# cnuns/Com-MARL

Hardware: AMD Instinct MI355X
Metric: env-steps/sec (whole node), PredatorPrey M=10 N=4, 4096 envs at 1/2/4/8 GPUs (higher is better)
Workload: dtype f32

## Files before the change

com-marl_amd/csrc/cm_env_pp10_dev.h:

```cpp
#pragma once
#include "cm_env_dev.h"

namespace cm {
namespace pp10 {

constexpr int S = 10, N = 4, M = 4, D = 21;
constexpr uint32_t ONES = 0x01010101u, HIGH = 0x80808080u, LOW7 = 0x7f7f7f7fu, SIXTEENS = 0x10101010u;

__device__ __forceinline__ uint32_t cell_of(int r, int c) { return (uint32_t)((r + 1) * 16 + c + 1); }
__device__ __forceinline__ int row_of(uint32_t ci) { return (int)(ci >> 4) - 1; }
__device__ __forceinline__ int col_of(uint32_t ci) { return (int)(ci & 15u) - 1; }
__device__ __forceinline__ uint32_t byte_at(uint32_t w, int i) { return (w >> (8 * i)) & 0xffu; }
__device__ __forceinline__ uint32_t set_byte(uint32_t w, int i, uint32_t v) { return (w & ~(0xffu << (8 * i))) | (v << (8 * i)); }
__device__ __forceinline__ uint32_t bcast(uint32_t t) { return t * ONES; }
__device__ __forceinline__ uint32_t any0(uint32_t x) { return (x - ONES) & ~x & HIGH; }
__device__ __forceinline__ uint32_t zero_bytes(uint32_t x) { return ~(((x & LOW7) + LOW7) | x | LOW7); }
__device__ __forceinline__ uint32_t delta_of(int a) { return (uint32_t)(16 * dr_of(a) + dc_of(a)); }
__device__ __forceinline__ int inside(uint32_t t) { return (((t >> 4) - 1u) < 10u) & (((t & 15u) - 1u) < 10u); }
__device__ __forceinline__ int lacks(uint32_t layer, uint32_t t) { return any0(layer ^ bcast(t)) == 0u; }
__device__ __forceinline__ uint32_t live_preys(uint32_t ppos, uint32_t flags) {
    uint32_t w = ppos;
#pragma unroll
    for (int j = 0; j < M; ++j) w |= ((flags >> j) & 1u) ? 0u : (0xffu << (8 * j));
    return w;
}
__device__ __forceinline__ int count_next(uint32_t layer, uint32_t t) {
    return __popc(zero_bytes(layer ^ bcast(t - 16u)) | zero_bytes(layer ^ bcast(t - 1u)) | zero_bytes(layer ^ bcast(t + 1u)) |
                  zero_bytes(layer ^ bcast(t + 16u)));
}
struct Shifted { uint32_t m16, m1, p1, p16; };
__device__ __forceinline__ int agents_next(const Shifted &a, uint32_t t) {
    const uint32_t bt = bcast(t);
    return __popc(zero_bytes(a.m16 ^ bt) | zero_bytes(a.m1 ^ bt) | zero_bytes(a.p1 ^ bt) | zero_bytes(a.p16 ^ bt));
}
__device__ __forceinline__ int no_agent_next(const Shifted &a, uint32_t t) {
    const uint32_t bt = bcast(t);
    return (any0(a.m16 ^ bt) | any0(a.m1 ^ bt) | any0(a.p1 ^ bt) | any0(a.p16 ^ bt)) == 0u;
}

struct State { uint32_t apos, ppos, flags; };
struct Pre { uint32_t rng_step; int step_count_in, succ; float t_rc, t_step0, t_step; double t_rew; };

__device__ __forceinline__ uint32_t elem_code(int k) {
    const int i = k / D, f = k - D * i;
    int x;
    if (f < 18) { const int chn = f >= 9, w = f - 9 * chn, wr = w / 3, wc = w - 3 * wr; x = (wr * 16 + wc) | (chn << 6); }
    else x = 35 + (f - 18);
    return (uint32_t)(i | (x << 2));
}
struct Emit { uint32_t e0, e1; };
__device__ __forceinline__ Emit emit_codes(int sl) {
    Emit e{ 0u, 0u };
#pragma unroll
    for (int u = 0; u < 6; ++u) {
        const int k = min(16 * u + sl, N * D - 1);
        const uint32_t c = elem_code(k) << (10 * (u % 3));
        if (u < 3) e.e0 |= c; else e.e1 |= c;
    }
    return e;
}

__device__ __forceinline__ State load_state(const EnvDev &p, int b) {
    State s{ 0u, 0u, 0u };
#pragma unroll
    for (int i = 0; i < N; ++i) {
        const int2 q = p.agent_pos[(size_t)b * N + i];
        s.apos |= cell_of(q.x, q.y) << (8 * i);
        s.flags |= (p.agent_cond[(size_t)b * N + i] != 0 ? 16u : 0u) << i;
    }
#pragma unroll
    for (int j = 0; j < M; ++j) {
        const int2 q = p.prey_pos[(size_t)b * M + j];
        s.ppos |= cell_of(q.x, q.y) << (8 * j);
        s.flags |= (p.alive[(size_t)b * M + j] != 0 ? 1u : 0u) << j;
    }
    return s;
}
__device__ __forceinline__ Pre load_pre(const EnvDev &p, int b, int sl, int tx) {
    Pre e;
    e.step_count_in = p.step_count[b];
    e.succ = p.success[b];
    e.rng_step = p.rng_step[b];
    const int s0 = sl < S ? sl : S - 1;
    e.t_rc = (tx & 16) ? p.lut_col[s0] : p.lut_row[s0];
    e.t_step0 = p.lut_step[0];
    e.t_rew = p.rew_lut[sl < (M + 1) + (N + 1) ? sl : 0];
    const int sc = e.step_count_in + 1;
    e.t_step = p.lut_step[sc <= p.max_steps ? sc : p.max_steps];
    return e;
}

struct StepOff { uint32_t obs, reward, reward_f64, done, details, prey_alive, success, path_len; };
template <class T>
__device__ __forceinline__ T *at32(T *base, uint32_t elem) { return reinterpret_cast<T *>(reinterpret_cast<char *>(base) + (uint32_t)(elem * (uint32_t)sizeof(T))); }

__device__ __forceinline__ void write_back(const EnvDev &p, uint32_t b, int sl, uint32_t apos, uint32_t ppos, uint32_t flags, int step_count,
                                           int succ, uint32_t rng_step) {
    if (sl == 0) {
        *at32(p.rng_step, b) = rng_step;
        *at32(p.step_count, b) = step_count;
        *at32(p.success, b) = succ;
    }
    if (sl < M) {
        const uint32_t ca = byte_at(apos, sl), cp = byte_at(ppos, sl);
        *at32(p.agent_pos, b * N + sl) = make_int2(row_of(ca), col_of(ca));
        *at32(p.prey_pos, b * M + sl) = make_int2(row_of(cp), col_of(cp));
        *at32(p.alive, b * M + sl) = (uint8_t)((flags >> sl) & 1u);
    }
}

__device__ __forceinline__ void step(const EnvDev &p, State &st, Pre &pre, const Emit em, int act_off, const cm_step_out &out,
                                     const StepOff &off, bool last, int grp, int b_raw, bool grp_live, int lds_base, bool all_valid,
                                     int obs_copy) {
    Grp<16> g;
    const int tx = thread_x();
    g.sub = (tx & (WAVE - 1)) / 16; g.sl = tx % 16;
    const int sl = g.sl;
    ENV_PROBE(0);
    const bool valid = all_valid || (grp_live && b_raw < p.B);
    const int b = valid ? b_raw : p.B - 1;
    const Rng rng{ (uint32_t)(p.env_id_offset + b), pre.rng_step, p.key0, p.key1 };
    const bool mine = sl < M;
    u32x4 x0 = { 0, 0, 0, 0 };
    if (mine) x0 = rng.at(SITE_PREY, (uint32_t)(2 * sl));
    const int4 araw = *reinterpret_cast<const int4 *>(smem + act_off);
    const int ain[4] = { araw.x, araw.y, araw.z, araw.w };
    int act[4], bad = 0;
#pragma unroll
    for (int i = 0; i < N; ++i) {
        const int a = ain[i];
        const int bi = (unsigned)a > 4u;
        bad |= bi;
        const int faulty = ((st.flags >> (4 + i)) & 1u) == 0u;
        act[i] = bi ? 4 : ((faulty & (a != 4)) ? 5 : a);
    }
    if (bad && valid) {
        if (sl == 0) raise(p, CM_ERR_ACTION);
        write_back(p, (uint32_t)b, sl, st.apos, st.ppos, st.flags, pre.step_count_in, pre.succ, pre.rng_step);
    }
    const bool commit = valid && !bad;
    ENV_PROBE(1);
    ENV_PROBE(2);

    uint32_t apos = st.apos, ppos = st.ppos, flags = st.flags;
    uint32_t plive = live_preys(ppos, flags);
    int moving = 0;
#pragma unroll
    for (int i = 0; i < N; ++i) {
        const int a = act[i];
        const int active = a != 4;
        moving += active;
        const uint32_t t = byte_at(apos, i) + delta_of(a);
        const int ok = active & inside(t) & lacks(apos, t) & lacks(plive, t);
        apos = ok ? set_byte(apos, i, t) : apos;
    }
    ENV_PROBE(3);
    const Shifted ag{ apos - SIXTEENS, apos - ONES, apos + ONES, apos + SIXTEENS };
    int pk;
    {
        const uint32_t my = byte_at(ppos, sl & 3);
        const int my_alive = mine & (int)((flags >> (sl & 3)) & 1u);
        const int cnt = my_alive ? agents_next(ag, my) : 0;
        int mv = 4;
        int found = (my_alive ^ 1) | ((p.load == 2) & (cnt >= 2));
#pragma unroll
        for (int t = 0; t < 4; ++t) {
            const int m = prey_move_from_u32(pick(x0, t));
            const int ok = no_agent_next(ag, my + delta_of(m)) & (found ^ 1);
            mv = ok ? m : mv; found |= ok;
        }
        if (!found) {
            const u32x4 x1 = rng.at(SITE_PREY, (uint32_t)(2 * sl + 1));
            const int m = prey_move_from_u32(x1.x);
            mv = no_agent_next(ag, my + delta_of(m)) ? m : mv;
        }
        pk = cnt | (mv << 3);
    }
    ENV_PROBE(8);
    const int wsum = g.count(mine && count_next(plive, byte_at(apos, sl & 3)) != 0);
    int pks[M];
#pragma unroll
    for (int j = 0; j < M; ++j) pks[j] = __shfl(pk, j, 16);
    ENV_PROBE(4);
    int capture = 0, penalty = 0, alive_any = 0;
#pragma unroll
    for (int j = 0; j < M; ++j) {
        const uint32_t c = byte_at(ppos, j);
        const int alive = (int)((flags >> j) & 1u), cnt = pks[j] & 7, mv = pks[j] >> 3;
        int need = p.load;
        if (p.load != 2) {
            const uint32_t rf = c >> 4, cf = c & 15u;
            const int on_r = (rf == 1u) | (rf == (uint32_t)S), on_c = (cf == 1u) | (cf == (uint32_t)S);
            const int adj = (on_r & on_c) ? 2 : ((on_r | on_c) ? 3 : p.load);
            const int avail = adj - count_next(plive, c);
            need = p.load < avail ? p.load : avail;
        }
        const int hit = alive & (cnt >= 1), captured = hit & (need <= cnt);
        capture += captured; penalty += hit & (captured ^ 1);
        const int stays = alive & (captured ^ 1);
        const uint32_t t = c + delta_of(mv);
        const int ok = stays & (mv != 4) & inside(t) & lacks(apos, t) & lacks(plive, t);
        ppos = ok ? set_byte(ppos, j, t) : ppos;
        plive = stays ? (ok ? set_byte(plive, j, t) : plive) : (plive | (0xffu << (8 * j)));
        flags = stays ? flags : (flags & ~(1u << j));
        alive_any |= stays;
    }
    ENV_PROBE(5);
    double reward = __shfl(pre.t_rew, capture, 16) + __shfl(pre.t_rew, (M + 1) + moving, 16);
    if (p.load == 2) reward = reward + p.penalty * (double)penalty;
    const cm_step_out &o = out;
    const uint32_t ub = (uint32_t)b;
    if (commit && mine) *at32(o.prey_alive, off.prey_alive + ub * M + sl) = (uint8_t)((flags >> sl) & 1u);
    int step_count = pre.step_count_in + 1, succ = pre.succ;
    int done = (step_count >= p.max_steps) || !alive_any;
    if (done) succ = alive_any ? 0 : 1;
    if (step_count >= p.mpl) done = 1;
    if (sl == 0 && commit) {
        *at32(o.reward, off.reward + ub) = (float)reward;
        *at32(o.reward_f64, off.reward_f64 + ub) = reward;
        *at32(o.done, off.done + ub) = (uint8_t)done;
        *at32(o.path_len, off.path_len + ub) = done ? step_count : 0;
        int2 *dd = reinterpret_cast<int2 *>(at32(o.details, off.details + ub * 6));
        dd[0] = make_int2(capture, moving); dd[1] = make_int2(penalty, 0); dd[2] = make_int2(wsum, 0);
    }
    ENV_PROBE(6);
    if (__any(done)) {
        const Lds l = make_lds(S, N, M, lds_base + p.lds_env * grp, p.status);
        do_reset<CM_PP, 16>(p, l, rng, cm_rng_tape{}, b, g, done != 0);
        if (done) {
            uint32_t a = 0u, q = 0u;
#pragma unroll
            for (int i = 0; i < N; ++i) { a |= cell_of(AR(l, i), AC(l, i)) << (8 * i); q |= cell_of(PR(l, i), PC(l, i)) << (8 * i); }
            apos = a; ppos = q;
            flags |= 0x0fu;
        }
    }
    if (done) step_count = 0;
    ENV_PROBE(7);
    const float t_clock = done ? pre.t_step0 : pre.t_step;
    plive = live_preys(ppos, flags);
    float vv[6];
    int ci_copy[6];
#pragma unroll
    for (int u = 0; u < 6; ++u) {
        const uint32_t code = ((u < 3 ? em.e0 : em.e1) >> (10 * (u % 3))) & 0x1ffu;
        const uint32_t i = code & 3u, x = code >> 2, w = x & 63u;
        const uint32_t ci = (apos >> (8u * i)) & 0xffu;
        const uint32_t t = ci + w - 17u;
        const int hit = !lacks((x & 64u) ? plive : apos, t);
        const float tab = __shfl(pre.t_rc, x == 36u ? 16 + col_of(ci) : row_of(ci), 64);
        vv[u] = w < 35u ? (hit ? 1.0f : 0.0f) : (x == 37u ? t_clock : tab);
        ci_copy[u] = 16 * u + sl + 3 * (int)i;
    }
    st.apos = apos; st.ppos = ppos; st.flags = (commit && done) ? (flags | 0xf0u) : flags;
    pre.rng_step += 1u;
    if (commit) { pre.step_count_in = step_count; pre.succ = succ; }
    {
        const int sc = pre.step_count_in + 1;
        pre.t_step = p.lut_step[sc <= p.max_steps ? sc : p.max_steps];
    }
    if (!commit) return;
    if (sl == 0) *at32(o.success, off.success + ub) = succ;
    const uint32_t ob = off.obs + ub * (N * D) + (uint32_t)sl;
    float *oc = reinterpret_cast<float *>(smem + obs_copy);
#pragma unroll
    for (int u = 0; u < 6; ++u) {
        if (16 * u + sl < N * D) {
            *at32(o.obs, ob + 16u * u) = vv[u];
            oc[ci_copy[u]] = vv[u];
        }
    }
    static_assert(OBS_COPY_STRIDE == D + 3, "the copy index k + 3i assumes rows of 24 floats");
    if (last) write_back(p, ub, sl, apos, ppos, flags, step_count, succ, rng.step + 1);
    ENV_PROBE(9);
}

}
}
```

com-marl_amd/csrc/cm_policy_w_dev.h:

```cpp
#pragma once
#include <type_traits>

#include "cm_policy_h_dev.h"

namespace cm {
namespace mw {

using mf::FwdArgs;
using mf::v4f;
using mf::fast_tanh;
using mf::EH; using mf::EMB; using mf::H1; using mf::H2; using mf::H3; using mf::MAX_ACT;
using mh::v8h; using mh::v4h; using mh::h16;

constexpr int WG_ENVS = 16, WG_ROWS = 64, KH = 32;
constexpr int FRAG = 64;

struct PackW { int enc1, enc2, attn, gcn, x1, h3, h4, bias, lds_u4, h2, total; };
__host__ __device__ constexpr int frag_u4(int K, int OUT) { return (OUT / 16) * (K / 32) * 2 * FRAG; }
constexpr int BIAS_U4 = 144;
__host__ __device__ constexpr PackW pack_w(int L) {
    PackW o{};
    int off = 0;
    o.enc1 = off; off += frag_u4(KH, EH);
    o.enc2 = off; off += frag_u4(EH, EMB);
    o.attn = off; off += frag_u4(EMB, EMB);
    o.gcn = off; off += L * frag_u4(EMB, EMB);
    o.x1 = off; off += frag_u4(EMB, H1);
    o.h3 = off; off += frag_u4(H2, H3);
    o.h4 = off; off += frag_u4(H3, 32);
    o.bias = off; off += BIAS_U4;
    o.lds_u4 = off;
    o.h2 = off; off += frag_u4(H1, H2);
    o.total = off;
    return o;
}

struct BiasMap { int e1, e2, g, b1, b2, b3, b4, total; };
__host__ __device__ constexpr BiasMap bias_map(int L) {
    BiasMap o{};
    int off = 0;
    o.e1 = off; off += EH; o.e2 = off; off += EMB; o.g = off; off += (L > 0 ? L : 1) * EMB;
    o.b1 = off; off += H1; o.b2 = off; off += H2; o.b3 = off; off += H3; o.b4 = off; off += 32;
    o.total = off;
    return o;
}
__host__ __device__ inline size_t lds_policy_bytes(int L) { return (size_t)pack_w(L).lds_u4 * 16 + WG_ROWS * 4; }

struct WeightsW {
    const uint4 *pack;
    int n_act;
};

__host__ __device__ inline int kmap(int q, int g, int e) { return 32 * q + 16 * (e >> 2) + 4 * g + (e & 3); }

template <int KB> struct Act { v8h hi[KB], lo[KB]; };

#define CM_MFW(A, B, ACC) ACC = __builtin_amdgcn_mfma_f32_16x16x32_f16(A, B, ACC, 0, 0, 0)

template <int KB, int CT>
struct Frags {
    v8h h[CT][KB], l[CT][KB];
    template <int TAG = 0>
    __device__ __forceinline__ void fetch(const uint4 *W, int lane) {
#pragma unroll
        for (int ct = 0; ct < CT; ++ct)
#pragma unroll
            for (int q = 0; q < KB; ++q) {
                h[ct][q] = __builtin_bit_cast(v8h, W[((ct * KB + q) * 2 + 0) * FRAG + lane]);
                l[ct][q] = __builtin_bit_cast(v8h, W[((ct * KB + q) * 2 + 1) * FRAG + lane]);
            }
        __builtin_amdgcn_sched_barrier(0);
    }
};

template <int CT, bool ON>
struct BiasR {
    v4f b[ON ? CT : 1];
    template <int C0 = 0>
    __device__ __forceinline__ void fetch(const float *bias, int g) {
        if constexpr (ON) {
#pragma unroll
            for (int ct = C0; ct < CT; ++ct) { const float4 v = *reinterpret_cast<const float4 *>(bias + 16 * ct + 4 * g); b[ct] = (v4f){ v.x, v.y, v.z, v.w }; }
            __builtin_amdgcn_sched_barrier(0);
        }
    }
    __device__ __forceinline__ const v4f *regs() const { return ON ? b : nullptr; }
};
struct NoHook { __device__ __forceinline__ void operator()() const {} };

constexpr float TANH_PRESCALE = 2.8853900817779268f;

template <int N>
__device__ __forceinline__ void tanh_stage(float (&v)[N]) {
    float e[N];
#pragma unroll
    for (int i = 0; i < N; ++i) e[i] = __builtin_amdgcn_exp2f(v[i]);
#pragma unroll
    for (int i = 0; i < N; ++i) e[i] += 1.0f;
#pragma unroll
    for (int i = 0; i < N; ++i) e[i] = __builtin_amdgcn_rcpf(e[i]);
#pragma unroll
    for (int i = 0; i < N; ++i) v[i] = fmaf(-2.0f, e[i], 1.0f);
}
typedef _Float16 v2h __attribute__((ext_vector_type(2)));
typedef float v2f __attribute__((ext_vector_type(2)));
__host__ __device__ inline void split_u(float x, h16 &h, h16 &l) { h = (h16)x; l = (h16)(x - (float)h); }
enum { SPLIT_SUB = 0, SPLIT_MIX = 1, SPLIT_MIXLO = 2 };
constexpr int SPLIT_DEFAULT = SPLIT_MIXLO;
__device__ __forceinline__ float opaque_minus_one() { float m; asm("s_mov_b32 %0, -1.0" : "=s"(m)); return m; }
template <int N, int MODE = SPLIT_DEFAULT>
__device__ __forceinline__ void split_stage(const float (&y)[N], h16 (&h)[N], h16 (&l)[N]) {
    static_assert(N % 2 == 0, "pairs");
    float d[N];
#pragma unroll
    for (int i = 0; i < N; i += 2) { const v2h p = __builtin_convertvector((v2f){ y[i], y[i + 1] }, v2h); h[i] = p[0]; h[i + 1] = p[1]; }
    if constexpr (MODE == SPLIT_MIXLO) {
        const float m1 = opaque_minus_one();
#pragma unroll
        for (int i = 0; i < N; ++i) l[i] = (h16)__builtin_fmaf((float)h[i], m1, y[i]);
        return;
    }
    if constexpr (MODE == SPLIT_MIX) {
        const float m1 = opaque_minus_one();
#pragma unroll
        for (int i = 0; i < N; ++i) d[i] = __builtin_fmaf((float)h[i], m1, y[i]);
    } else {
#pragma unroll
        for (int i = 0; i < N; ++i) d[i] = y[i] - (float)h[i];
    }
#pragma unroll
    for (int i = 0; i < N; i += 2) { const v2h p = __builtin_convertvector((v2f){ d[i], d[i + 1] }, v2h); l[i] = p[0]; l[i + 1] = p[1]; }
}

template <int KB, int CT, bool TANH, bool BIAS, int SPLIT = SPLIT_DEFAULT, int PB0 = CT, class MID = NoHook>
__device__ __forceinline__ void dense_act(const Frags<KB, CT> &f, const float *bias, const Act<KB> &x, Act<CT / 2> &y, v4f *keep, int lane,
                                          float *sv = nullptr, const v4f *pb = nullptr, MID mid = MID{}) {
    const int g = lane >> 4;
    const v4f zero = (v4f){ 0.f, 0.f, 0.f, 0.f };
    v4f acc[CT];
#pragma unroll
    for (int p = 0; p <= CT / 2; ++p) {
        if constexpr (!std::is_same<MID, NoHook>::value) { if (p == CT / 4) mid(); }
        if (p < CT / 2) {
#pragma unroll
            for (int t = 0; t < 2; ++t) {
                const int ct = 2 * p + t;
                if (BIAS && ct >= PB0) acc[ct] = pb[ct];
                else if (BIAS) { const float4 b = *reinterpret_cast<const float4 *>(bias + 16 * ct + 4 * g); acc[ct] = (v4f){ b.x, b.y, b.z, b.w }; }
#pragma unroll
                for (int q = 0; q < KB; ++q) {
                    const v4f a0 = (q == 0 && !BIAS) ? zero : acc[ct];
                    acc[ct] = __builtin_amdgcn_mfma_f32_16x16x32_f16(f.h[ct][q], x.lo[q], a0, 0, 0, 0);
                    acc[ct] = __builtin_amdgcn_mfma_f32_16x16x32_f16(f.l[ct][q], x.hi[q], acc[ct], 0, 0, 0);
                    acc[ct] = __builtin_amdgcn_mfma_f32_16x16x32_f16(f.h[ct][q], x.hi[q], acc[ct], 0, 0, 0);
                }
            }
        }
        if (p > 0) {
            float v[8];
#pragma unroll
            for (int e = 0; e < 8; ++e) v[e] = acc[2 * (p - 1) + (e >> 2)][e & 3];
            if (TANH) tanh_stage<8>(v);
            if (keep) {
#pragma unroll
                for (int e = 0; e < 8; ++e) keep[2 * (p - 1) + (e >> 2)][e & 3] = v[e];
            }
            if (sv) {
                *reinterpret_cast<float4 *>(sv + 16 * (2 * (p - 1)) + 4 * g) = make_float4(v[0], v[1], v[2], v[3]);
                *reinterpret_cast<float4 *>(sv + 16 * (2 * (p - 1) + 1) + 4 * g) = make_float4(v[4], v[5], v[6], v[7]);
            }
            h16 h[8], l[8];
            split_stage<8, SPLIT>(v, h, l);
#pragma unroll
            for (int e = 0; e < 8; ++e) { y.hi[p - 1][e] = h[e]; y.lo[p - 1][e] = l[e]; }
        }
    }
}

template <int KB, int CT, bool SWAP, bool BIAS, bool PREB = false>
__device__ __forceinline__ void dense_f32(const Frags<KB, CT> &f, const float *bias, const Act<KB> &x, v4f (&out)[CT], int lane, const v4f *pb = nullptr) {
    const int g = lane >> 4;
    const v4f zero = (v4f){ 0.f, 0.f, 0.f, 0.f };
#pragma unroll
    for (int ct = 0; ct < CT; ++ct) {
        v4f acc = zero;
        if constexpr (BIAS && PREB) acc = pb[ct];
        else if (BIAS) { const float4 b = *reinterpret_cast<const float4 *>(bias + 16 * ct + 4 * g); acc = (v4f){ b.x, b.y, b.z, b.w }; }
#pragma unroll
        for (int q = 0; q < KB; ++q) {
            if (!SWAP) {
                acc = __builtin_amdgcn_mfma_f32_16x16x32_f16(f.h[ct][q], x.lo[q], acc, 0, 0, 0);
                acc = __builtin_amdgcn_mfma_f32_16x16x32_f16(f.l[ct][q], x.hi[q], acc, 0, 0, 0);
                acc = __builtin_amdgcn_mfma_f32_16x16x32_f16(f.h[ct][q], x.hi[q], acc, 0, 0, 0);
            } else {
                acc = __builtin_amdgcn_mfma_f32_16x16x32_f16(x.lo[q], f.h[ct][q], acc, 0, 0, 0);
                acc = __builtin_amdgcn_mfma_f32_16x16x32_f16(x.hi[q], f.l[ct][q], acc, 0, 0, 0);
                acc = __builtin_amdgcn_mfma_f32_16x16x32_f16(x.hi[q], f.h[ct][q], acc, 0, 0, 0);
            }
        }
        out[ct] = acc;
    }
}

#define CM_WPROBE(i) do { if (a.probe && tid == 0) a.probe[(size_t)blk * mf::NPROBE + (i)] = __builtin_amdgcn_s_memtime(); } while (0)

template <int LHOPS>
__device__ __forceinline__ void stage_w(const WeightsW &w, unsigned char *lds, int tid) {
    constexpr PackW pk = pack_w(LHOPS);
    uint4 *WL = reinterpret_cast<uint4 *>(lds);
    constexpr int PER = (pk.lds_u4 + 255) / 256, BATCH = (PER + 1) / 2;
    const int rot = (int)((blockIdx.x * 7u) % (unsigned)(2 * BATCH));
    auto chunk_of = [&](int j) { const int c = j + rot; return c >= 2 * BATCH ? c - 2 * BATCH : c; };
#pragma unroll
    for (int round = 0; round < 2; ++round) {
        uint4 v[BATCH];
#pragma unroll
        for (int k = 0; k < BATCH; ++k) { const int i = chunk_of(round * BATCH + k) * 256 + tid; v[k] = w.pack[i < pk.lds_u4 ? i : 0]; }
#pragma unroll
        for (int k = 0; k < BATCH; ++k) { const int i = chunk_of(round * BATCH + k) * 256 + tid; if (i < pk.lds_u4) WL[i] = v[k]; }
    }
}

template <bool LEAN = false>
struct ResidentW {
    Frags<4, 4> h2;
    struct None {};
    std::conditional_t<LEAN, Frags<2, 2>, None> h3;
    std::conditional_t<LEAN, Frags<1, 2>, None> h4;
    template <class R, class F>
    static __device__ __forceinline__ const F &pick(const R &resident, const F &own) { if constexpr (LEAN) return resident; else return own; }
    template <int LHOPS>
    __device__ __forceinline__ void fetch(const WeightsW &w, int lane) {
        h2.template fetch<LEAN>(w.pack + pack_w(LHOPS).h2, lane);
        if constexpr (LEAN) {
            h3.template fetch<LEAN>(w.pack + pack_w(LHOPS).h3, lane);
            h4.template fetch<LEAN>(w.pack + pack_w(LHOPS).h4, lane);
#pragma unroll
            for (int ct = 0; ct < 2; ++ct) {
#pragma unroll
                for (int q = 0; q < 2; ++q) { asm volatile("" : "+a"(h3.h[ct][q])); asm volatile("" : "+a"(h3.l[ct][q])); }
                asm volatile("" : "+a"(h4.h[ct][0])); asm volatile("" : "+a"(h4.l[ct][0]));
            }
        }
#pragma unroll
        for (int ct = 0; ct < 4; ++ct)
#pragma unroll
            for (int q = 0; q < 4; ++q) { asm volatile("" : "+a"(h2.h[ct][q])); asm volatile("" : "+a"(h2.l[ct][q])); }
    }
};

struct StepOff { uint32_t actions, probs, attn; };
template <class T>
__device__ __forceinline__ T *at32(T *base, uint32_t elem) { return reinterpret_cast<T *>(reinterpret_cast<char *>(base) + (uint32_t)(elem * (uint32_t)sizeof(T))); }
template <int LHOPS, bool OBS_LDS = false, bool TRAIN = false, int HEADK = 0, bool STEP32 = false, bool LEAN = false>
__device__ __forceinline__ void policy_tile_w(const FwdArgs &a, int n_act, const ResidentW<LEAN> &res, const unsigned char *lds, int blk,
                                              int32_t *act_lds, int obs_row = 0, const StepOff so = StepOff{}) {
    static_assert(!STEP32 || (!TRAIN && HEADK == 0), "step offsets: the acting forward of the rollout");
    static_assert(!LEAN || (!TRAIN && HEADK == 0), "the lean tile: the acting forward of the rollout");
    constexpr int E1H = LEAN ? 4 : 8, E2H = LEAN ? 2 : 4;
    constexpr int PB_H2 = LEAN ? 0 : 4, PB_H3 = LEAN ? 0 : 2;
    static_assert(HEADK == 0 || TRAIN, "the critic head exists as training forward only");
    static_assert(LHOPS >= 1 && LHOPS <= 2, "wave-owned forward: one or two hops");
    const int tid = thread_x(), wave = tid >> 6, lane = tid & 63, c = lane & 15, g = lane >> 4;
    constexpr PackW pk = pack_w(LHOPS);
    constexpr BiasMap bm = bias_map(LHOPS);
    const uint4 *WL = reinterpret_cast<const uint4 *>(lds);
    const float *BL = reinterpret_cast<const float *>(lds + (size_t)pk.bias * 16);
    const int s0 = blk * WG_ENVS;
    const int row = wave * 16 + c;
    const size_t grow = (size_t)s0 * 4 + row;
    const int env_l = wave * 4 + (c >> 2), agent = c & 3;
    const bool diag = g == (c >> 2);
    const bool rv = s0 + env_l < a.S;

    CM_WPROBE(2);
    Act<1> xo;
    {
        float ov[8];
        if constexpr (OBS_LDS) {
            const float4 *src = reinterpret_cast<const float4 *>(lds + obs_row + 32 * (g < 3 ? g : 0));
            const float4 v0 = src[0], v1 = src[1];
            const float vv[8] = { v0.x, v0.y, v0.z, v0.w, v1.x, v1.y, v1.z, v1.w };
#pragma unroll
            for (int e = 0; e < 8; ++e) ov[e] = (rv && g < 3) ? vv[e] : 0.0f;
        } else {
        const float *src = a.obs + (rv ? grow : 0) * a.d;
#pragma unroll
        for (int e = 0; e < 8; ++e) { const int k = 8 * g + e; const float v = src[k < a.d ? k : 0]; ov[e] = (rv && k < a.d) ? v : 0.0f; }
        }
        h16 h[8], l[8];
        split_stage<8>(ov, h, l);
#pragma unroll
        for (int e = 0; e < 8; ++e) { xo.hi[0][e] = h[e]; xo.lo[0][e] = l[e]; }
    }
    const uint32_t draw_step = a.policy_step + (a.step_base ? *a.step_base : 0u);

    Frags<1, 8> f_e1; f_e1.template fetch<LEAN>(WL + pk.enc1, lane);
    BiasR<8, LEAN> r_e1;
    Frags<4, 4> f_e2;
    if constexpr (!LEAN) f_e2.template fetch<LEAN>(WL + pk.enc2, lane);
    auto sv_row = [&](float *base, int width) -> float * { return (TRAIN && base && rv) ? base + grow * (size_t)width : nullptr; };
    Act<4> a1;
    if constexpr (LEAN)
        dense_act<1, 8, true, true, SPLIT_DEFAULT, E1H>(f_e1, BL + bm.e1, xo, a1, nullptr, lane, nullptr, r_e1.regs(),
                                                        [&] { r_e1.template fetch<E1H>(BL + bm.e1, g); f_e2.template fetch<LEAN>(WL + pk.enc2, lane); });
    else dense_act<1, 8, true, true>(f_e1, BL + bm.e1, xo, a1, nullptr, lane, sv_row(a.sv_a1, EH));
    BiasR<4, LEAN> r_e2;
    Frags<2, 4> f_at;
    if constexpr (!LEAN) f_at.template fetch<LEAN>(WL + pk.attn, lane);
    v4f E[4];
    Act<2> xe;
    if constexpr (LEAN)
        dense_act<4, 4, true, true, SPLIT_DEFAULT, E2H>(f_e2, BL + bm.e2, a1, xe, E, lane, nullptr, r_e2.regs(),
                                                        [&] { r_e2.template fetch<E2H>(BL + bm.e2, g); f_at.template fetch<LEAN>(WL + pk.attn, lane); });
    else dense_act<4, 4, true, true>(f_e2, BL + bm.e2, a1, xe, E, lane, sv_row(a.sv_e, EMB));
    Frags<2, 4> f_g; f_g.template fetch<LEAN>(WL + pk.gcn, lane);
    CM_WPROBE(3);

    float m[4];
    {
        Act<2> xq;
        dense_act<2, 4, false, false>(f_at, nullptr, xe, xq, nullptr, lane, sv_row(a.sv_q, EMB));
        v4f hh = (v4f){ 0.f, 0.f, 0.f, 0.f };
#pragma unroll
        for (int q = 0; q < 2; ++q) { CM_MFW(xe.hi[q], xq.lo[q], hh); CM_MFW(xe.lo[q], xq.hi[q], hh); CM_MFW(xe.hi[q], xq.hi[q], hh); }
        float sc[4], mx = -INFINITY, sum = 0.0f;
#pragma unroll
        for (int r = 0; r < 4; ++r) { sc[r] = hh[r]; mx = fmaxf(mx, sc[r]); }
#pragma unroll
        for (int r = 0; r < 4; ++r) { m[r] = __builtin_amdgcn_exp2f((sc[r] - mx) * 1.4426950408889634f); sum += m[r]; }
        const float rs = __builtin_amdgcn_rcpf(sum);
#pragma unroll
        for (int r = 0; r < 4; ++r) m[r] *= rs;
    }
    const size_t env_g = (size_t)s0 + env_l;
    if (a.attn && diag && rv) {
        float *dst = STEP32 ? at32(a.attn, so.attn + (uint32_t)env_g * 16u + 4u * (uint32_t)agent) : a.attn + env_g * 16 + 4 * agent;
        __builtin_nontemporal_store(m[0], dst); __builtin_nontemporal_store(m[1], dst + 1);
        __builtin_nontemporal_store(m[2], dst + 2); __builtin_nontemporal_store(m[3], dst + 3);
    }

    CM_WPROBE(5);
    Act<2> xh = xe;
    Frags<2, HEADK == 0 ? 8 : 4> f_x1;
    BiasR<8, LEAN> r_b1;
    BiasR<4, LEAN> r_b2;
    BiasR<2, LEAN> r_b3;
    BiasR<2, LEAN> r_b4;
#pragma unroll
    for (int l = 0; l < LHOPS; ++l) {
        v4f hw[4];
        dense_f32<2, 4, true, false>(f_g, nullptr, xh, hw, lane);
        if constexpr (TRAIN) {
            if (a.sv_hw[l] && s0 + wave * 4 + g < a.S) {
                float *dst = a.sv_hw[l] + ((size_t)s0 * 4 + wave * 16 + 4 * g) * EMB + c;
#pragma unroll
                for (int ct = 0; ct < 4; ++ct)
#pragma unroll
                    for (int r = 0; r < 4; ++r) dst[(size_t)r * EMB + 16 * ct] = hw[ct][r] * (1.0f / TANH_PRESCALE);
            }
        }
        BiasR<4, LEAN> r_g; r_g.fetch(BL + bm.g + l * EMB, g);
        if (l + 1 < LHOPS) f_g.template fetch<LEAN>(WL + pk.gcn + (l + 1) * frag_u4(EMB, EMB), lane);
        else {
            r_b1.fetch(BL + bm.b1, g);
            f_x1.template fetch<LEAN>(WL + pk.x1, lane);
        }
        float cf[4], den = 0.0f;
#pragma unroll
        for (int r = 0; r < 4; ++r) {
            float x = m[r];
            if (a.adj && rv) x *= a.adj[env_g * 16 + 4 * agent + r];
            if (a.chan && rv) x *= a.chan[(env_g * LHOPS + l) * 16 + 4 * agent + r];
            cf[r] = x; den += x;
        }
        const float rden = __builtin_amdgcn_rcpf(den + 1e-12f);
        v4h bh, bl;
        {
            float cn[4];
            h16 h[4], lo_[4];
#pragma unroll
            for (int r = 0; r < 4; ++r) cn[r] = diag ? cf[r] * rden : 0.0f;
            split_stage<4>(cn, h, lo_);
#pragma unroll
            for (int r = 0; r < 4; ++r) { bh[r] = h[r]; bl[r] = lo_[r]; }
        }
        const bool last = l == LHOPS - 1;
        v4h ah[4], al[4];
        {
            float hv[16];
            h16 h[16], lo_[16];
#pragma unroll
            for (int i = 0; i < 16; ++i) hv[i] = hw[i >> 2][i & 3];
            split_stage<16>(hv, h, lo_);
#pragma unroll
            for (int i = 0; i < 16; ++i) { ah[i >> 2][i & 3] = h[i]; al[i >> 2][i & 3] = lo_[i]; }
        }
        v4f acc[4];
#pragma unroll
        for (int ct = 0; ct < 4; ++ct) {
            v4f b0;
            if constexpr (LEAN) b0 = r_g.b[ct];
            else { const float4 b = *reinterpret_cast<const float4 *>(BL + bm.g + l * EMB + 16 * ct + 4 * g); b0 = (v4f){ b.x, b.y, b.z, b.w }; }
            acc[ct] = __builtin_amdgcn_mfma_f32_16x16x16f16(ah[ct], bl, b0, 0, 0, 0);
            acc[ct] = __builtin_amdgcn_mfma_f32_16x16x16f16(al[ct], bh, acc[ct], 0, 0, 0);
            acc[ct] = __builtin_amdgcn_mfma_f32_16x16x16f16(ah[ct], bh, acc[ct], 0, 0, 0);
        }
#pragma unroll
        for (int p = 0; p < 2; ++p) {
            float v[8];
#pragma unroll
            for (int e = 0; e < 8; ++e) v[e] = acc[2 * p + (e >> 2)][e & 3];
            tanh_stage<8>(v);
            if (last && !a.no_residual) {
#pragma unroll
                for (int e = 0; e < 8; ++e) v[e] += E[2 * p + (e >> 2)][e & 3];
            }
            if constexpr (TRAIN) {
                if (float *sv = sv_row(a.sv_h[l], EMB)) {
                    *reinterpret_cast<float4 *>(sv + 16 * (2 * p) + 4 * g) = make_float4(v[0], v[1], v[2], v[3]);
                    *reinterpret_cast<float4 *>(sv + 16 * (2 * p + 1) + 4 * g) = make_float4(v[4], v[5], v[6], v[7]);
                }
            }
            h16 h[8], lo_[8];
            split_stage<8>(v, h, lo_);
#pragma unroll
            for (int e = 0; e < 8; ++e) { xh.hi[p][e] = h[e]; xh.lo[p][e] = lo_[e]; }
        }
    }

    CM_WPROBE(6);
    if constexpr (HEADK == 1) {
        Frags<2, 1> f_d2; f_d2.template fetch<LEAN>(WL + pk.h3, lane);
        Act<2> xd;
        dense_act<2, 4, true, true>(f_x1, BL + bm.b1, xh, xd, nullptr, lane, sv_row(a.sv_x1, EMB));
        v4f val[1];
        dense_f32<2, 1, false, true>(f_d2, BL + bm.b2, xd, val, lane);
        float v = (g == 0 && rv) ? val[0][0] : 0.0f;
        if (a.sv_out && g == 0 && rv) a.sv_out[grow] = v;
        v += __shfl_xor(v, 1);
        v += __shfl_xor(v, 2);
        if (a.values && g == 0 && rv && agent == 0) a.values[(size_t)s0 + env_l] = v;
        return;
    } else {
    Act<4> x1;
    if constexpr (LEAN) {
        dense_act<2, 8, true, true, SPLIT_DEFAULT, 0>(f_x1, BL + bm.b1, xh, x1, nullptr, lane, nullptr, r_b1.regs(),
                                                      [&] { r_b2.fetch(BL + bm.b2, g); r_b3.fetch(BL + bm.b3, g); r_b4.fetch(BL + bm.b4, g); });
    } else dense_act<2, 8, true, true>(f_x1, BL + bm.b1, xh, x1, nullptr, lane, sv_row(a.sv_x1, H1));
    Frags<2, 2> f_h3_lds;
    Frags<1, 2> f_h4_lds;
    if constexpr (!LEAN) { f_h3_lds.template fetch<LEAN>(WL + pk.h3, lane); f_h4_lds.template fetch<LEAN>(WL + pk.h4, lane); }
    const Frags<2, 2> &f_h3 = res.pick(res.h3, f_h3_lds);
    const Frags<1, 2> &f_h4 = res.pick(res.h4, f_h4_lds);
    float u = 0.0f;
    if constexpr (!TRAIN) {
        const u32x4 xr = philox4x32_10((uint32_t)(a.env_id_offset + (int)env_g), draw_step, SITE_ACTION, (uint32_t)agent, a.key0, a.key1);
        u = unit_f32(xr.x);
    }
    CM_WPROBE(7);
    Act<2> x2;
    dense_act<4, 4, true, true, SPLIT_DEFAULT, PB_H2>(res.h2, BL + bm.b2, x1, x2, nullptr, lane, sv_row(a.sv_x2, H2), r_b2.regs());
    Act<1> x3;
    dense_act<2, 2, true, true, SPLIT_DEFAULT, PB_H3>(f_h3, BL + bm.b3, x2, x3, nullptr, lane, sv_row(a.sv_x3, H3), r_b3.regs());
    v4f lg[2];
    dense_f32<1, 2, false, true, LEAN>(f_h4, BL + bm.b4, x3, lg, lane, r_b4.regs());

    CM_WPROBE(9);
    const int A = n_act;
    float p[MAX_ACT];
#pragma unroll
    for (int cc = 0; cc < MAX_ACT; ++cc) p[cc] = cc < 4 ? lg[0][cc] : (cc == 4 ? lg[1][0] : 0.0f);
    if constexpr (TRAIN) {
        if (a.sv_out && g == 0 && rv) {
#pragma unroll
            for (int cc = 0; cc < 5; ++cc) if (cc < A) a.sv_out[grow * A + cc] = p[cc];
        }
    }
    float mx = -INFINITY, sum = 0.0f, msum = 0.0f;
#pragma unroll
    for (int cc = 0; cc < 5; ++cc) if (cc < A) mx = fmaxf(mx, p[cc]);
#pragma unroll
    for (int cc = 0; cc < 5; ++cc) if (cc < A) { p[cc] = __builtin_amdgcn_exp2f((p[cc] - mx) * 1.4426950408889634f); sum += p[cc]; }
    const float rsum = __builtin_amdgcn_rcpf(sum);
#pragma unroll
    for (int cc = 0; cc < 5; ++cc) if (cc < A) {
        const float av = (a.avail && rv) ? a.avail[grow * A + cc] : 1.0f;
        p[cc] = (p[cc] * rsum) * av; msum += p[cc];
    }
    const float rmsum = __builtin_amdgcn_rcpf(msum);
#pragma unroll
    for (int cc = 0; cc < 5; ++cc) if (cc < A) p[cc] = p[cc] * rmsum;
    if (g == 0 && rv) {
        if (a.probs) {
#pragma unroll
            for (int cc = 0; cc < 5; ++cc) if (cc < A)
                __builtin_nontemporal_store(p[cc], STEP32 ? at32(a.probs, so.probs + (uint32_t)grow * (uint32_t)A + cc) : a.probs + grow * A + cc);
        }
        if (a.actions || act_lds) {
            int act = 0;
            if (a.greedy) {
                float best = p[0];
#pragma unroll
                for (int cc = 1; cc < 5; ++cc) if (cc < A && p[cc] > best) { best = p[cc]; act = cc; }
            } else {
                float acc = 0.0f;
                int sel = -1, lastc = 0;
#pragma unroll
                for (int cc = 0; cc < 5; ++cc) if (cc < A) { if (p[cc] > 0.0f) lastc = cc; acc += p[cc]; if (sel < 0 && u < acc) sel = cc; }
                act = sel < 0 ? lastc : sel;
            }
            if (a.actions) *(STEP32 ? at32(a.actions, so.actions + (uint32_t)grow) : a.actions + grow) = act;
            if (act_lds) act_lds[row] = act;
        }
    }
    }
    CM_WPROBE(10);
}
#undef CM_MFW

template <int LHOPS>
__device__ __forceinline__ void fwd_body_w(const FwdArgs &a, const WeightsW &w, unsigned char *lds, int blk, int32_t *act_lds) {
    const int tid = thread_x();
    CM_WPROBE(0);
    stage_w<LHOPS>(w, lds, tid);
    ResidentW<> res;
    res.fetch<LHOPS>(w, tid & 63);
    CM_WPROBE(1);
    __syncthreads();
    policy_tile_w<LHOPS>(a, w.n_act, res, lds, blk, act_lds);
}

__host__ inline bool shape_ok_w(int N, int d, int L, int n_act) { return N == 4 && d <= KH && (L == 1 || L == 2) && n_act >= 1 && n_act <= 5; }

}
}
```

com-marl_amd/csrc/cm_rollout_w_body.h:

```cpp
    static_assert(SHAPE == 0 || CARRY, "shape constants are built into the carried form only");
    if constexpr (SHAPE == 1) {
        p.S = 10; p.M = 4; p.R = 1; p.W = 3; p.d = 21; p.rcp_d = 1.0f / 21.0f; p.rcp_W = 1.0f / 3.0f; p.rcp_WW = 1.0f / 9.0f;
        p.lds_env = lds_env_bytes(10, 4, 4);
        a.N = 4; a.d = 21; a.L = LHOPS;
        a.avail = nullptr; a.greedy = 0; a.adj = nullptr; a.chan = nullptr; a.probe = nullptr;
        __builtin_assume(a.actions != nullptr); __builtin_assume(a.probs != nullptr); __builtin_assume(a.attn != nullptr);
        if constexpr (!PROBES) p.stop = 0;
    }
    const int n_act = SHAPE == 1 ? 5 : w.n_act;
    static_assert(!CARRY || (PRE && !TAPE), "the carried form is the prefetching, tape-less build");
    const cm_rng_tape tape = TAPE ? tape_arg : cm_rng_tape{};
    if constexpr (!TAPE) p.rng_mode = CM_RNG_PHILOX;
    p.scen = CM_PP; p.N = 4; p.lpe = 16; p.rcp_N = 0.25f; p.rcp_NN = 0.0625f;
    if constexpr (CARRY) { p.adj_const = 1; p.ch_const = 1; p.channel = CM_CH_FC; }
    extern __shared__ __attribute__((aligned(16))) unsigned char lds_w[];
    constexpr int LPE = 16;
    constexpr int ACT_OFF = mw::pack_w(LHOPS).lds_u4 * 16, ENV_BASE = ACT_OFF + mw::WG_ROWS * 4;
    int32_t *act = reinterpret_cast<int32_t *>(lds_w + ACT_OFF);
    const bool probe = PROBES && p.stop == -2 && blockIdx.x == 0 && thread_x() == 0;
    const unsigned long long t_in = probe ? __builtin_amdgcn_s_memtime() : 0ull;
    mw::stage_w<LHOPS>(w, lds_w, thread_x());
    mw::ResidentW<SHAPE == 1> res;
    res.template fetch<LHOPS>(w, thread_x() & 63);
    __syncthreads();
    if (probe) { g_w_probe[3] = __builtin_amdgcn_s_memtime() - t_in; g_w_probe[0] = g_w_probe[1] = g_w_probe[2] = g_w_probe[4] = 0; }
    const int envs = FULLWG ? mw::WG_ENVS : min(mw::WG_ENVS, a.S - (int)blockIdx.x * mw::WG_ENVS);
    EnvPre pre{};
    pp10::State st{};
    pp10::Pre pp{};
    pp10::Emit em{};
    int obs_row = 0, obs_env = -1;
    if constexpr (CARRY) {
        const int tx = thread_x(), grp = tx / LPE, lane = tx & 63, cc = lane & 15;
        const bool live = FULLWG || grp < envs;
        const Lds l0 = make_lds(p.S, p.N, p.M, ENV_BASE + p.lds_env * grp, p.status);
        obs_env = l0.win;
        const int env_l = (tx >> 6) * 4 + (cc >> 2);
        obs_row = make_lds(p.S, p.N, p.M, ENV_BASE + p.lds_env * env_l, p.status).win + (cc & 3) * OBS_COPY_STRIDE * 4;
        float *oc = reinterpret_cast<float *>(lds_w + obs_env);
        const int b0 = blockIdx.x * mw::WG_ENVS + (live ? grp : 0);
        const bool ok = live && b0 < a.S;
        for (int k = tx % LPE; k < 4 * OBS_COPY_STRIDE; k += LPE) {
            const int i = k / OBS_COPY_STRIDE, f = k - i * OBS_COPY_STRIDE;
            oc[k] = (ok && f < a.d) ? a.obs[((size_t)b0 * 4 + i) * a.d + f] : 0.0f;
        }
        if constexpr (SHAPE == 1) {
            const int b = (live && b0 < p.B) ? b0 : p.B - 1;
            st = pp10::load_state(p, b);
            pp = pp10::load_pre(p, b, tx % LPE, tx);
            em = pp10::emit_codes(tx % LPE);
        } else pre = env_prefetch<CM_PP, LPE>(p, b0, live);
    }
    for (int t = 0; t < c.n_steps; ++t) {
        asm volatile("" ::: "memory");
        const int tx = thread_x(), grp = tx / LPE;
        const bool live = FULLWG || grp < envs;
        const bool env_wave = FULLWG || (tx & ~63) / LPE < envs;
        const int b_raw = blockIdx.x * mw::WG_ENVS + (live ? grp : 0);
        mf::FwdArgs at = a;
        at.policy_step = a.policy_step + (uint32_t)t;
        const uint32_t ut = (uint32_t)t;
        if constexpr (SHAPE != 1) {
        at.obs = a.obs + (size_t)t * c.obs;
        at.adj = a.adj ? a.adj + (size_t)t * c.dist_adj : nullptr;
        at.chan = a.chan ? a.chan + (size_t)t * c.channels : nullptr;
        at.actions = a.actions ? a.actions + (size_t)t * c.actions : nullptr;
        at.probs = a.probs ? a.probs + (size_t)t * c.probs : nullptr;
        at.attn = a.attn ? a.attn + (size_t)t * c.attn : nullptr;
        }
        const unsigned long long t0 = probe ? __builtin_amdgcn_s_memtime() : 0ull;
        if constexpr (PRE && !CARRY) pre = env_prefetch<CM_PP, LPE>(p, b_raw, live);
        if constexpr (SHAPE == 1)
            mw::policy_tile_w<LHOPS, true, false, 0, true, true>(at, n_act, res, lds_w, blockIdx.x, act, obs_row,
                                                           mw::StepOff{ ut * (uint32_t)c.actions, ut * (uint32_t)c.probs, ut * (uint32_t)c.attn });
        else mw::policy_tile_w<LHOPS, CARRY>(at, n_act, res, lds_w, blockIdx.x, act, obs_row);
        asm volatile("s_waitcnt lgkmcnt(0)" ::: "memory");
        const unsigned long long t1 = probe ? __builtin_amdgcn_s_memtime() : 0ull;
        cm_step_out ot = out;
        if constexpr (SHAPE != 1) {
        if (ot.obs) ot.obs += (size_t)t * c.obs;
        if (ot.reward) ot.reward += (size_t)t * c.reward;
        if (ot.reward_f64) ot.reward_f64 += (size_t)t * c.reward_f64;
        if (ot.done) ot.done += (size_t)t * c.done;
        if (ot.details) ot.details += (size_t)t * c.details;
        if (ot.dist_adj) ot.dist_adj += (size_t)t * c.dist_adj;
        if (ot.channels) ot.channels += (size_t)t * c.channels;
        if (ot.prey_alive) ot.prey_alive += (size_t)t * c.prey_alive;
        if (ot.success) ot.success += (size_t)t * c.success;
        if (ot.path_len) ot.path_len += (size_t)t * c.path_len;
        }
        if (env_wave) {
            const int32_t *my_act = act + (live ? grp : 0) * 4;
            if constexpr (CARRY && SHAPE == 1) {
                const pp10::StepOff so{ ut * (uint32_t)c.obs, ut * (uint32_t)c.reward, ut * (uint32_t)c.reward_f64, ut * (uint32_t)c.done,
                                        ut * (uint32_t)c.details, ut * (uint32_t)c.prey_alive, ut * (uint32_t)c.success, ut * (uint32_t)c.path_len };
                pp10::step(p, st, pp, em, ACT_OFF + (live ? grp : 0) * 16, ot, so, t == c.n_steps - 1, grp, b_raw, live, ENV_BASE, FULLWG, obs_env);
            } else if constexpr (CARRY) {
                const bool bad = env_stage<CM_PP, LPE>(p, pre, my_act, grp, ENV_BASE);
                EnvCarry carry{ pre.step_count_in, pre.succ, 0 };
                env_body<CM_PP, LPE>(p, nullptr, my_act, tape, ot, 0, grp, b_raw, live, ENV_BASE, nullptr, true, pre.rng_step, pre.step_count_in,
                                     pre.succ, pre.t_row, pre.t_col, pre.t_step0, pre.t_step, pre.t_rew, bad, FULLWG, &carry, obs_env);
                pre = env_pre_carry<CM_PP, LPE>(p, pre, carry, grp, ENV_BASE);
            } else if constexpr (PRE) {
                const bool bad = env_stage<CM_PP, LPE>(p, pre, my_act, grp, ENV_BASE);
                env_body<CM_PP, LPE>(p, nullptr, my_act, tape, ot, 0, grp, b_raw, live, ENV_BASE, nullptr, true, pre.rng_step, pre.step_count_in,
                                     pre.succ, pre.t_row, pre.t_col, pre.t_step0, pre.t_step, pre.t_rew, bad, FULLWG);
            } else env_body<CM_PP, LPE>(p, nullptr, my_act, tape, ot, 0, grp, b_raw, live, ENV_BASE);
        }
        const unsigned long long tf = probe ? __builtin_amdgcn_s_memtime() : 0ull;
        if constexpr (!CARRY) {
            __builtin_amdgcn_fence(__ATOMIC_RELEASE, "workgroup");
            __builtin_amdgcn_fence(__ATOMIC_ACQUIRE, "workgroup");
        }
        if (probe) { const unsigned long long t2 = __builtin_amdgcn_s_memtime(); g_w_probe[0] += 1; g_w_probe[1] += t1 - t0; g_w_probe[2] += t2 - t1; g_w_probe[4] += t2 - tf; }
    }
    if constexpr (CARRY) {
        if (tl.on) {
            const int tx = thread_x(), grp = tx / LPE, sl = tx % LPE;
            const int b0 = blockIdx.x * mw::WG_ENVS + grp;
            if ((FULLWG || grp < envs) && b0 < a.S) {
                const float *oc = reinterpret_cast<const float *>(lds_w + obs_env);
                float *dst = tl.obs_dst + (size_t)b0 * 4 * a.d;
                const float rcp_d = p.rcp_d;
                for (int k = sl; k < 4 * a.d; k += LPE) { const int i = fdiv(k, a.d, rcp_d), f = k - i * a.d; dst[k] = oc[i * OBS_COPY_STRIDE + f]; }
            }
            if ((tx & 63) == 0) {
                const unsigned int last = gridDim.x * (blockDim.x >> 6) - 1;
                if (atomicAdd(tl.ticket, 1u) == last) { *tl.base += (uint32_t)c.n_steps; *tl.ticket = 0u; }
            }
        }
    }
```

Before: 435.1 million.

## Batch Philox draws for prey moves and action sampling into one per-wave stage

Adds a draw stage in which every lane of a wave computes one Philox block, for either a prey-move draw or an action-sampling draw covering two steps, and stores it in LDS. The policy tile and the env step then read their random words from that buffer instead of each computing Philox on only a subset of lanes. The buffer reuses the h3/h4 weight slots, which are no longer staged for this shape, and the step base is folded into policy_step once. This fills idle lanes and removes duplicated RNG work, at the risk of LDS aliasing errors and a change in RNG counter semantics.

New measurement: 448.2 million, median of 6. +3.0%, better.

```diff
diff --git a/com-marl_amd/csrc/cm_env_pp10_dev.h b/com-marl_amd/csrc/cm_env_pp10_dev.h
--- a/com-marl_amd/csrc/cm_env_pp10_dev.h
+++ b/com-marl_amd/csrc/cm_env_pp10_dev.h
@@ -109,9 +109,35 @@
     }
 }
 
+__device__ __forceinline__ void draw_stage(const EnvDev &p, uint32_t rng_step, int32_t act_gid0, uint32_t act_step, uint32_t act_k0,
+                                           uint32_t act_k1, int envs, bool all_valid, int buf) {
+    const int tx = thread_x(), lane = tx & (WAVE - 1), idx = lane & 15;
+    const bool prey = (lane & 16) != 0;
+    const uint32_t half = (uint32_t)(lane >> 5);
+    const int tgt = (tx >> 6) * 4 + (idx >> 2);
+    const int b_raw = blockIdx.x * 16 + tgt;
+    const bool valid = all_valid || (tgt < envs && b_raw < p.B);
+    const int b = valid ? b_raw : p.B - 1;
+    const uint32_t rs = (uint32_t)__shfl((int)rng_step, (idx >> 2) * 16, WAVE);
+    uint32_t c0 = prey ? (uint32_t)(p.env_id_offset + b) : (uint32_t)(act_gid0 + b_raw);
+    uint32_t c1 = (prey ? rs : act_step) + half;
+    uint32_t c2 = prey ? (uint32_t)SITE_PREY : (uint32_t)SITE_ACTION;
+    uint32_t c3 = prey ? 2u * (uint32_t)(idx & 3) : (uint32_t)(idx & 3);
+    uint32_t k0 = prey ? p.key0 : act_k0, k1 = prey ? p.key1 : act_k1;
+#pragma unroll
+    for (int r = 0; r < 10; ++r) {
+        const uint64_t p0 = (uint64_t)0xD2511F53u * c0, p1 = (uint64_t)0xCD9E8D57u * c2;
+        const uint32_t n0 = (uint32_t)(p1 >> 32) ^ c1 ^ k0, n1 = (uint32_t)p1;
+        const uint32_t n2 = (uint32_t)(p0 >> 32) ^ c3 ^ k1, n3 = (uint32_t)p0;
+        c0 = n0; c1 = n1; c2 = n2; c3 = n3;
+        k0 += 0x9E3779B9u; k1 += 0xBB67AE85u;
+    }
+    *reinterpret_cast<uint4 *>(smem + buf + 16 * lane) = make_uint4(c0, c1, c2, c3);
+}
+
 __device__ __forceinline__ void step(const EnvDev &p, State &st, Pre &pre, const Emit em, int act_off, const cm_step_out &out,
                                      const StepOff &off, bool last, int grp, int b_raw, bool grp_live, int lds_base, bool all_valid,
-                                     int obs_copy) {
+                                     int obs_copy, int draw) {
     Grp<16> g;
     const int tx = thread_x();
     g.sub = (tx & (WAVE - 1)) / 16; g.sl = tx % 16;
@@ -121,8 +147,9 @@
     const int b = valid ? b_raw : p.B - 1;
     const Rng rng{ (uint32_t)(p.env_id_offset + b), pre.rng_step, p.key0, p.key1 };
     const bool mine = sl < M;
-    u32x4 x0 = { 0, 0, 0, 0 };
-    if (mine) x0 = rng.at(SITE_PREY, (uint32_t)(2 * sl));
+    const uint2 *dq = reinterpret_cast<const uint2 *>(smem + draw + 16 * (4 * g.sub + (sl & 3)));
+    const uint2 d01 = dq[0], d23 = dq[1];
+    const u32x4 x0 = { d01.x, d01.y, d23.x, d23.y };
     const int4 araw = *reinterpret_cast<const int4 *>(smem + act_off);
     const int ain[4] = { araw.x, araw.y, araw.z, araw.w };
     int act[4], bad = 0;
diff --git a/com-marl_amd/csrc/cm_policy_w_dev.h b/com-marl_amd/csrc/cm_policy_w_dev.h
--- a/com-marl_amd/csrc/cm_policy_w_dev.h
+++ b/com-marl_amd/csrc/cm_policy_w_dev.h
@@ -45,6 +45,9 @@
     return o;
 }
 __host__ __device__ inline size_t lds_policy_bytes(int L) { return (size_t)pack_w(L).lds_u4 * 16 + WG_ROWS * 4; }
+constexpr int DRAW_WAVE_BYTES = 64 * 16;
+__host__ __device__ constexpr int draw_lds_off(int L) { return pack_w(L).h3 * 16; }
+static_assert((pack_w(1).bias - pack_w(1).h3) * 16 >= (WG_ROWS / 16) * DRAW_WAVE_BYTES, "the draw buffer lies inside the h3 / h4 slots");
 
 struct WeightsW {
     const uint4 *pack;
@@ -204,20 +207,21 @@
 
 #define CM_WPROBE(i) do { if (a.probe && tid == 0) a.probe[(size_t)blk * mf::NPROBE + (i)] = __builtin_amdgcn_s_memtime(); } while (0)
 
-template <int LHOPS>
+template <int LHOPS, bool NO_HEAD = false>
 __device__ __forceinline__ void stage_w(const WeightsW &w, unsigned char *lds, int tid) {
     constexpr PackW pk = pack_w(LHOPS);
     uint4 *WL = reinterpret_cast<uint4 *>(lds);
     constexpr int PER = (pk.lds_u4 + 255) / 256, BATCH = (PER + 1) / 2;
     const int rot = (int)((blockIdx.x * 7u) % (unsigned)(2 * BATCH));
     auto chunk_of = [&](int j) { const int c = j + rot; return c >= 2 * BATCH ? c - 2 * BATCH : c; };
+    auto staged = [&](int i) { return i < pk.lds_u4 && !(NO_HEAD && i >= pk.h3 && i < pk.bias); };
 #pragma unroll
     for (int round = 0; round < 2; ++round) {
         uint4 v[BATCH];
 #pragma unroll
-        for (int k = 0; k < BATCH; ++k) { const int i = chunk_of(round * BATCH + k) * 256 + tid; v[k] = w.pack[i < pk.lds_u4 ? i : 0]; }
-#pragma unroll
-        for (int k = 0; k < BATCH; ++k) { const int i = chunk_of(round * BATCH + k) * 256 + tid; if (i < pk.lds_u4) WL[i] = v[k]; }
+        for (int k = 0; k < BATCH; ++k) { const int i = chunk_of(round * BATCH + k) * 256 + tid; v[k] = w.pack[staged(i) ? i : 0]; }
+#pragma unroll
+        for (int k = 0; k < BATCH; ++k) { const int i = chunk_of(round * BATCH + k) * 256 + tid; if (staged(i)) WL[i] = v[k]; }
     }
 }
 
@@ -254,7 +258,7 @@
 __device__ __forceinline__ T *at32(T *base, uint32_t elem) { return reinterpret_cast<T *>(reinterpret_cast<char *>(base) + (uint32_t)(elem * (uint32_t)sizeof(T))); }
 template <int LHOPS, bool OBS_LDS = false, bool TRAIN = false, int HEADK = 0, bool STEP32 = false, bool LEAN = false>
 __device__ __forceinline__ void policy_tile_w(const FwdArgs &a, int n_act, const ResidentW<LEAN> &res, const unsigned char *lds, int blk,
-                                              int32_t *act_lds, int obs_row = 0, const StepOff so = StepOff{}) {
+                                              int32_t *act_lds, int obs_row = 0, const StepOff so = StepOff{}, int draw_off = 0) {
     static_assert(!STEP32 || (!TRAIN && HEADK == 0), "step offsets: the acting forward of the rollout");
     static_assert(!LEAN || (!TRAIN && HEADK == 0), "the lean tile: the acting forward of the rollout");
     constexpr int E1H = LEAN ? 4 : 8, E2H = LEAN ? 2 : 4;
@@ -293,7 +297,8 @@
 #pragma unroll
         for (int e = 0; e < 8; ++e) { xo.hi[0][e] = h[e]; xo.lo[0][e] = l[e]; }
     }
-    const uint32_t draw_step = a.policy_step + (a.step_base ? *a.step_base : 0u);
+    uint32_t draw_step = 0u;
+    if constexpr (!LEAN) draw_step = a.policy_step + (a.step_base ? *a.step_base : 0u);
 
     Frags<1, 8> f_e1; f_e1.template fetch<LEAN>(WL + pk.enc1, lane);
     BiasR<8, LEAN> r_e1;
@@ -454,7 +459,7 @@
     const Frags<2, 2> &f_h3 = res.pick(res.h3, f_h3_lds);
     const Frags<1, 2> &f_h4 = res.pick(res.h4, f_h4_lds);
     float u = 0.0f;
-    if constexpr (!TRAIN) {
+    if constexpr (!TRAIN && !LEAN) {
         const u32x4 xr = philox4x32_10((uint32_t)(a.env_id_offset + (int)env_g), draw_step, SITE_ACTION, (uint32_t)agent, a.key0, a.key1);
         u = unit_f32(xr.x);
     }
@@ -464,6 +469,7 @@
     Act<1> x3;
     dense_act<2, 2, true, true, SPLIT_DEFAULT, PB_H3>(f_h3, BL + bm.b3, x2, x3, nullptr, lane, sv_row(a.sv_x3, H3), r_b3.regs());
     v4f lg[2];
+    if constexpr (LEAN) u = unit_f32(*reinterpret_cast<const uint32_t *>(lds + draw_off + 16 * c));
     dense_f32<1, 2, false, true, LEAN>(f_h4, BL + bm.b4, x3, lg, lane, r_b4.regs());
 
     CM_WPROBE(9);
diff --git a/com-marl_amd/csrc/cm_rollout_w_body.h b/com-marl_amd/csrc/cm_rollout_w_body.h
--- a/com-marl_amd/csrc/cm_rollout_w_body.h
+++ b/com-marl_amd/csrc/cm_rollout_w_body.h
@@ -6,6 +6,8 @@
         a.avail = nullptr; a.greedy = 0; a.adj = nullptr; a.chan = nullptr; a.probe = nullptr;
         __builtin_assume(a.actions != nullptr); __builtin_assume(a.probs != nullptr); __builtin_assume(a.attn != nullptr);
         if constexpr (!PROBES) p.stop = 0;
+        a.policy_step += a.step_base ? *a.step_base : 0u;
+        a.step_base = nullptr;
     }
     const int n_act = SHAPE == 1 ? 5 : w.n_act;
     static_assert(!CARRY || (PRE && !TAPE), "the carried form is the prefetching, tape-less build");
@@ -16,10 +18,11 @@
     extern __shared__ __attribute__((aligned(16))) unsigned char lds_w[];
     constexpr int LPE = 16;
     constexpr int ACT_OFF = mw::pack_w(LHOPS).lds_u4 * 16, ENV_BASE = ACT_OFF + mw::WG_ROWS * 4;
+    constexpr int DRAW_OFF = mw::draw_lds_off(LHOPS);
     int32_t *act = reinterpret_cast<int32_t *>(lds_w + ACT_OFF);
     const bool probe = PROBES && p.stop == -2 && blockIdx.x == 0 && thread_x() == 0;
     const unsigned long long t_in = probe ? __builtin_amdgcn_s_memtime() : 0ull;
-    mw::stage_w<LHOPS>(w, lds_w, thread_x());
+    mw::stage_w<LHOPS, SHAPE == 1>(w, lds_w, thread_x());
     mw::ResidentW<SHAPE == 1> res;
     res.template fetch<LHOPS>(w, thread_x() & 63);
     __syncthreads();
@@ -69,10 +72,15 @@
         at.attn = a.attn ? a.attn + (size_t)t * c.attn : nullptr;
         }
         const unsigned long long t0 = probe ? __builtin_amdgcn_s_memtime() : 0ull;
+        const int draw = DRAW_OFF + __builtin_amdgcn_readfirstlane(tx >> 6) * mw::DRAW_WAVE_BYTES + (t & 1) * (mw::DRAW_WAVE_BYTES / 2);
+        if constexpr (SHAPE == 1) {
+            if ((t & 1) == 0) pp10::draw_stage(p, pp.rng_step, a.env_id_offset, at.policy_step, a.key0, a.key1, envs, FULLWG, draw);
+            asm volatile("" ::: "memory");
+        }
         if constexpr (PRE && !CARRY) pre = env_prefetch<CM_PP, LPE>(p, b_raw, live);
         if constexpr (SHAPE == 1)
             mw::policy_tile_w<LHOPS, true, false, 0, true, true>(at, n_act, res, lds_w, blockIdx.x, act, obs_row,
-                                                           mw::StepOff{ ut * (uint32_t)c.actions, ut * (uint32_t)c.probs, ut * (uint32_t)c.attn });
+                                                           mw::StepOff{ ut * (uint32_t)c.actions, ut * (uint32_t)c.probs, ut * (uint32_t)c.attn }, draw);
         else mw::policy_tile_w<LHOPS, CARRY>(at, n_act, res, lds_w, blockIdx.x, act, obs_row);
         asm volatile("s_waitcnt lgkmcnt(0)" ::: "memory");
         const unsigned long long t1 = probe ? __builtin_amdgcn_s_memtime() : 0ull;
@@ -94,7 +102,7 @@
             if constexpr (CARRY && SHAPE == 1) {
                 const pp10::StepOff so{ ut * (uint32_t)c.obs, ut * (uint32_t)c.reward, ut * (uint32_t)c.reward_f64, ut * (uint32_t)c.done,
                                         ut * (uint32_t)c.details, ut * (uint32_t)c.prey_alive, ut * (uint32_t)c.success, ut * (uint32_t)c.path_len };
-                pp10::step(p, st, pp, em, ACT_OFF + (live ? grp : 0) * 16, ot, so, t == c.n_steps - 1, grp, b_raw, live, ENV_BASE, FULLWG, obs_env);
+                pp10::step(p, st, pp, em, ACT_OFF + (live ? grp : 0) * 16, ot, so, t == c.n_steps - 1, grp, b_raw, live, ENV_BASE, FULLWG, obs_env, draw + mw::DRAW_WAVE_BYTES / 4);
             } else if constexpr (CARRY) {
                 const bool bad = env_stage<CM_PP, LPE>(p, pre, my_act, grp, ENV_BASE);
                 EnvCarry carry{ pre.step_count_in, pre.succ, 0 };
```
